# SmoothKen/knn-svc

Measured on AMD Instinct MI355X. Metric: audio-sec converted/sec (xRT) end-to-end, cold target pool, higher is better.
Workload: dtype f32; 1 GPU; north-star point per rank: 30 s source vs 10 min target pool (20 x 30 s), ckpt_type=mix, post_opt_0.2, cold (pool encoded inside the step); seeded random weights of WavLM-Large (6 layers executed) and the 22.9 M-param generator; nq=1500, np_per_rank=30000, wavlm_batch_chunks=32, pipeline_depth=2

## Files before the change

### knn_svc_amd/csrc/attention.hip

```cpp
#include "common.h"
#include "gemm2_core.h"
#include <stdlib.h>

namespace {

constexpr int HD = 64;
constexpr int KT = 64;
constexpr int LDKK = 68;
constexpr int LDV = 64;

__global__ __launch_bounds__(256) void attention_kernel(const float* __restrict__ qkv, const float* __restrict__ gate,
                                                       const float* __restrict__ table, const int* __restrict__ kv_len, int T, int heads,
                                                       float* __restrict__ out) {
    extern __shared__ __attribute__((aligned(16))) float lds[];
    float* Ks = lds;
    float* Vs = Ks + KT * LDKK;
    float* tb = Vs + KT * LDV;

    const int tid = threadIdx.x, lane = tid & 63, wave = tid >> 6;
    const int li = lane & 31, lh = lane >> 5;
    const int head = blockIdx.y, b = blockIdx.z;
    const int E = heads * HD;
    const long ld = 3L * E;
    const float* base = qkv + (long)b * T * ld;
// ... 240 lines not shown
                s = __builtin_amdgcn_mfma_f32_32x32x16_bf16(k0, q2, s, 0, 0, 0);
                s = __builtin_amdgcn_mfma_f32_32x32x16_bf16(k1, q0, s, 0, 0, 0);
                s = __builtin_amdgcn_mfma_f32_32x32x16_bf16(k0, q1, s, 0, 0, 0);
                s = __builtin_amdgcn_mfma_f32_32x32x16_bf16(k0, q0, s, 0, 0, 0);
            }
            const l_f* tp = tbq + kbase;
#pragma unroll
            for (int r = 0; r < 16; ++r) s[r] = fmaf(g_i, tp[(r & 3) + 8 * (r >> 2)], s[r]);
            if (kbase + 32 > Tk) {
#pragma unroll
                for (int r = 0; r < 16; ++r)
                    if (kbase + (r & 3) + 8 * (r >> 2) + 4 * lh >= Tk) s[r] = -__builtin_inff();
            }
            float mx = fmaxf(fmaxf(s[0], s[1]), fmaxf(s[2], s[3]));
#pragma unroll
            for (int r = 4; r < 16; r += 4) mx = fmaxf(mx, fmaxf(fmaxf(s[r], s[r + 1]), fmaxf(s[r + 2], s[r + 3])));
            mx = fmaxf(mx, __shfl_xor(mx, 32, 64));
            const float m_new = fmaxf(m_run, mx);
            const float alpha = __builtin_amdgcn_exp2f(m_run - m_new);
            float ps = 0.f;
#pragma unroll
            for (int r = 0; r < 16; ++r) { s[r] = __builtin_amdgcn_exp2f(s[r] - m_new); ps += s[r]; }
            ps += __shfl_xor(ps, 32, 64);
            l_run = l_run * alpha + ps;
            m_run = m_new;
            if (__builtin_amdgcn_ballot_w64(alpha != 1.f)) {
#pragma unroll
                for (int d = 0; d < 2; ++d)
#pragma unroll
                    for (int r = 0; r < 16; ++r) o[d][r] *= alpha;
            }
#pragma unroll
            for (int st = 0; st < 2; ++st) {
                unsigned h[8], m[8], l[8];
#pragma unroll
                for (int e = 0; e < 8; ++e) split3(s[8 * st + e], h[e], m[e], l[e]);
                au32x4 p0, p1, p2;
#pragma unroll
                for (int w = 0; w < 4; ++w) {
                    p0[w] = pack_hi(h[2 * w + 1], h[2 * w]); p1[w] = pack_hi(m[2 * w + 1], m[2 * w]); p2[w] = pack_hi(l[2 * w + 1], l[2 * w]);
                }
                const bf16x8_t b0 = __builtin_bit_cast(bf16x8_t, p0), b1 = __builtin_bit_cast(bf16x8_t, p1), b2 = __builtin_bit_cast(bf16x8_t, p2);
                const int kcol = (sub * 32 + 16 * st + 4 * lh) * 2;
#pragma unroll
                for (int dt = 0; dt < 2; ++dt) {
                    const lc* vp = Vs + (dt * 32 + li) * VP3 + kcol;
                    au32x4 a0, a1, a2;
                    const au32x2 x0 = *(const l_u2*)(vp), x1 = *(const l_u2*)(vp + 16);
                    const au32x2 y0 = *(const l_u2*)(vp + 128), y1 = *(const l_u2*)(vp + 128 + 16);
                    const au32x2 z0 = *(const l_u2*)(vp + 256), z1 = *(const l_u2*)(vp + 256 + 16);
                    a0 = (au32x4){x0[0], x0[1], x1[0], x1[1]};
                    a1 = (au32x4){y0[0], y0[1], y1[0], y1[1]};
                    a2 = (au32x4){z0[0], z0[1], z1[0], z1[1]};
                    const bf16x8_t v0 = __builtin_bit_cast(bf16x8_t, a0), v1 = __builtin_bit_cast(bf16x8_t, a1), v2 = __builtin_bit_cast(bf16x8_t, a2);
                    f32x16 c = o[dt];
                    c = __builtin_amdgcn_mfma_f32_32x32x16_bf16(v1, b1, c, 0, 0, 0);
                    c = __builtin_amdgcn_mfma_f32_32x32x16_bf16(v2, b0, c, 0, 0, 0);
                    c = __builtin_amdgcn_mfma_f32_32x32x16_bf16(v0, b2, c, 0, 0, 0);
                    c = __builtin_amdgcn_mfma_f32_32x32x16_bf16(v1, b0, c, 0, 0, 0);
                    c = __builtin_amdgcn_mfma_f32_32x32x16_bf16(v0, b1, c, 0, 0, 0);
                    c = __builtin_amdgcn_mfma_f32_32x32x16_bf16(v0, b0, c, 0, 0, 0);
                    o[dt] = c;
                }
            }
        }
    }
    if (qvalid) {
        const float inv = 1.0f / l_run;
        float* op = out + ((long)b * T + qi) * E + head * HD;
#pragma unroll
        for (int d = 0; d < 2; ++d)
#pragma unroll
            for (int r4 = 0; r4 < 4; ++r4) {
                f32x4 v = {o[d][r4 * 4 + 0] * inv, o[d][r4 * 4 + 1] * inv, o[d][r4 * 4 + 2] * inv, o[d][r4 * 4 + 3] * inv};
                *(f32x4*)(op + d * 32 + r4 * 8 + lh * 4) = v;
            }
    }
}

typedef short short4v __attribute__((ext_vector_type(4)));
constexpr int KP2 = 272;
constexpr int VP2 = 320;

__global__ __launch_bounds__(256, 3) void attention2_kernel(const float* __restrict__ qkv, const float* __restrict__ gate,
                                                           const float* __restrict__ table, const int* __restrict__ kv_len, int T, int heads,
                                                           float* __restrict__ out, int out_split, int kv_split) {
    extern __shared__ __attribute__((aligned(16))) float lds[];
    typedef __attribute__((address_space(3))) char lc;
    typedef __attribute__((address_space(3))) au32x4 l_u4;
    typedef __attribute__((address_space(3))) au32x2 l_u2;
    typedef __attribute__((address_space(3))) float l_f;
    lc* Ks = (lc*)lds;
    lc* Vs = Ks + KT * KP2;
    l_f* tb = (l_f*)(Vs + KT * VP2);

    const int tid = threadIdx.x, lane = tid & 63, wave = tid >> 6;
    const int li = lane & 31, lh = lane >> 5;
    const int head = blockIdx.y, b = blockIdx.z;
    const int E = heads * HD;
    const long ld = 3L * E;
    const float* base = qkv + (long)b * T * ld;
    const int qi = blockIdx.x * 128 + wave * 32 + li;
    const bool qvalid = qi < T;
    int Tk = T;
    if (kv_len) { Tk = kv_len[b]; Tk = Tk < 1 ? 1 : (Tk > T ? T : Tk); }

    for (int i = tid; i < 2 * T - 1 + 64; i += 256) tb[i] = i < 2 * T - 1 ? table[(long)head * (2 * T - 1) + i] : 0.f;

    const float L2E = 1.44269504088896341f;
    const float qscale = 0.125f * L2E * 16.0f;
    au32x4 qf[4][2];
#pragma unroll
    for (int s = 0; s < 4; ++s) {
        f32x4 v0 = {0.f, 0.f, 0.f, 0.f}, v1 = v0;
        if (qvalid) {
            const float* p = base + (long)qi * ld + head * HD + s * 16 + lh * 8;
            v0 = *(const f32x4*)p; v1 = *(const f32x4*)(p + 4);
        }
        g2_u32x2 h0, l0, h1, l1;
        f16x2_split4(v0, qscale, h0, l0); f16x2_split4(v1, qscale, h1, l1);
        qf[s][0] = (au32x4){h0[0], h0[1], h1[0], h1[1]};
        qf[s][1] = (au32x4){l0[0], l0[1], l1[0], l1[1]};
    }
    const float g_i = qvalid ? gate[((long)b * T + qi) * heads + head] * (L2E * 256.0f) : 0.f;
    const l_f* tbq = tb + (T - 1 - (qvalid ? qi : T - 1)) + 4 * lh;
    const lc* v_tr = Vs + (4 * (lane >> 5) + ((lane & 15) >> 2)) * VP2 + (16 * ((lane >> 4) & 1) + 4 * (lane & 3)) * 2;


    f32x16 o[2];
#pragma unroll
    for (int d = 0; d < 2; ++d)
#pragma unroll
        for (int r = 0; r < 16; ++r) o[d][r] = 0.f;
    float m_run = -__builtin_inff(), l_run = 0.f;

    const int srow = tid >> 4, scol = (tid & 15) * 4;
    f32x4 rk[4], rv[4];
    auto gload = [&](int k0) {
#pragma unroll
        for (int j = 0; j < 4; ++j) {
            const int key = k0 + srow + 16 * j;
            f32x4 kk = {0.f, 0.f, 0.f, 0.f}, vv = {0.f, 0.f, 0.f, 0.f};
            if (key < T) {
                const float* p = base + (long)key * ld + head * HD + scol;
                kk = *(const f32x4*)(p + E);
                vv = *(const f32x4*)(p + 2 * E);
            }
            rk[j] = kk; rv[j] = vv;
        }
    };
    gload(0);
    const int ntiles = (Tk + KT - 1) / KT;
    for (int t = 0; t < ntiles; ++t) {
#ifdef KN_ATT_NOSTAGE
        if (t == 0) {
#endif
        __syncthreads();
        if (kv_split) {
            const int pc = tid & 15, plane = (pc >> 2) & 1, d0 = (pc >> 3) * 32 + (pc & 3) * 8;
#pragma unroll
            for (int j = 0; j < 4; ++j) {
                const int key = srow + 16 * j;
                *(l_u4*)(Ks + key * KP2 + plane * 128 + d0 * 2) = __builtin_bit_cast(au32x4, rk[j]);
                *(l_u4*)(Vs + key * VP2 + plane * 128 + d0 * 2) = __builtin_bit_cast(au32x4, rv[j]);
            }
        } else {
#pragma unroll
        for (int j = 0; j < 4; ++j) {
            const int key = srow + 16 * j;
            g2_u32x2 hi, lo;
            f16x2_split4(rk[j], 16.0f, hi, lo);
            lc* kd = Ks + key * KP2 + scol * 2;
            *(l_u2*)(kd) = hi;
            *(l_u2*)(kd + 128) = lo;
            f16x2_split4(rv[j], 16.0f, hi, lo);
            lc* vd = Vs + key * VP2 + scol * 2;
            *(l_u2*)(vd) = hi;
            *(l_u2*)(vd + 128) = lo;
        }
        }
        __syncthreads();
#ifdef KN_ATT_NOSTAGE
        }
#else
        if (t + 1 < ntiles) gload((t + 1) * KT);
#endif

#pragma unroll
        for (int sub = 0; sub < 2; ++sub) {
            const int kbase = t * KT + sub * 32;
            if (kbase >= Tk) break;
            f32x16 s;
#pragma unroll
            for (int r = 0; r < 16; ++r) s[r] = 0.f;
            const lc* kp = Ks + (sub * 32 + li) * KP2 + lh * 16;
#pragma unroll
            for (int st = 0; st < 4; ++st) {
                const f16x8 k0 = __builtin_bit_cast(f16x8, *(const l_u4*)(kp + st * 32));
                const f16x8 k1 = __builtin_bit_cast(f16x8, *(const l_u4*)(kp + 128 + st * 32));
                const f16x8 q0 = __builtin_bit_cast(f16x8, qf[st][0]), q1 = __builtin_bit_cast(f16x8, qf[st][1]);
#ifdef KN_ATT_NOS
                if (st == 0) s = __builtin_amdgcn_mfma_f32_32x32x16_f16(k1, q0, s, 0, 0, 0);
                else { s[st] += __builtin_bit_cast(float, __builtin_bit_cast(au32x4, k0)[0] ^ __builtin_bit_cast(au32x4, k1)[1] ^ __builtin_bit_cast(au32x4, q1)[0]); }
#else
                s = __builtin_amdgcn_mfma_f32_32x32x16_f16(k1, q0, s, 0, 0, 0);
                s = __builtin_amdgcn_mfma_f32_32x32x16_f16(k0, q1, s, 0, 0, 0);
                s = __builtin_amdgcn_mfma_f32_32x32x16_f16(k0, q0, s, 0, 0, 0);
#endif
            }
            const l_f* tp = tbq + kbase;
#ifndef KN_ATT_NOBIAS
#pragma unroll
            for (int r = 0; r < 16; ++r) s[r] = fmaf(g_i, tp[(r & 3) + 8 * (r >> 2)], s[r]);
#endif
            if (kbase + 32 > Tk) {
#pragma unroll
                for (int r = 0; r < 16; ++r)
                    if (kbase + (r & 3) + 8 * (r >> 2) + 4 * lh >= Tk) s[r] = -__builtin_inff();
            }
#ifdef KN_ATT_NOEXP
            float mx = s[0];
#else
            float mx = fmaxf(fmaxf(s[0], s[1]), fmaxf(s[2], s[3]));
#pragma unroll
            for (int r = 4; r < 16; r += 4) mx = fmaxf(mx, fmaxf(fmaxf(s[r], s[r + 1]), fmaxf(s[r + 2], s[r + 3])));
#endif
            mx = fmaxf(mx, __shfl_xor(mx, 32, 64));
            const float m_new = fmaxf(m_run, mx);
            const float alpha = __builtin_amdgcn_exp2f((m_run - m_new) * (1.0f / 256.0f));
            const float mneg = fmaf(m_new, -1.0f / 256.0f, 14.0f);
            float ps = 0.f;
#pragma unroll
#ifdef KN_ATT_NOEXP
            for (int r = 0; r < 16; ++r) { s[r] = s[r] * 1e-9f; } ps = s[3] + mneg;
#else
            for (int r = 0; r < 16; ++r) { s[r] = __builtin_amdgcn_exp2f(fmaf(s[r], 1.0f / 256.0f, mneg)); ps += s[r]; }
#endif
            ps += __shfl_xor(ps, 32, 64);
            l_run = l_run * alpha + ps;
            m_run = m_new;
            if (__builtin_amdgcn_ballot_w64(alpha != 1.f)) {
#pragma unroll
                for (int d = 0; d < 2; ++d)
#pragma unroll
                    for (int r = 0; r < 16; ++r) o[d][r] *= alpha;
            }
#pragma unroll
            for (int st = 0; st < 2; ++st) {
                g2_u32x2 h0, l0, h1, l1;
                f16x2_split4((f32x4){s[8 * st + 0], s[8 * st + 1], s[8 * st + 2], s[8 * st + 3]}, 1.0f, h0, l0);
                f16x2_split4((f32x4){s[8 * st + 4], s[8 * st + 5], s[8 * st + 6], s[8 * st + 7]}, 1.0f, h1, l1);
                const f16x8 b0 = __builtin_bit_cast(f16x8, (au32x4){h0[0], h0[1], h1[0], h1[1]});
                const f16x8 b1 = __builtin_bit_cast(f16x8, (au32x4){l0[0], l0[1], l1[0], l1[1]});
                const lc* vrow = v_tr + (sub * 32 + 16 * st) * VP2;
#pragma unroll
                for (int dt = 0; dt < 2; ++dt) {
                    typedef __attribute__((address_space(3))) short4v l_s4;
                    const lc* vp = vrow + dt * 64;
                    const au32x2 x0 = __builtin_bit_cast(au32x2, __builtin_amdgcn_ds_read_tr16_b64_v4i16((l_s4*)(vp)));
                    const au32x2 x1 = __builtin_bit_cast(au32x2, __builtin_amdgcn_ds_read_tr16_b64_v4i16((l_s4*)(vp + 8 * VP2)));
                    const au32x2 y0 = __builtin_bit_cast(au32x2, __builtin_amdgcn_ds_read_tr16_b64_v4i16((l_s4*)(vp + 128)));
                    const au32x2 y1 = __builtin_bit_cast(au32x2, __builtin_amdgcn_ds_read_tr16_b64_v4i16((l_s4*)(vp + 8 * VP2 + 128)));
                    const f16x8 v0 = __builtin_bit_cast(f16x8, (au32x4){x0[0], x0[1], x1[0], x1[1]});
                    const f16x8 v1 = __builtin_bit_cast(f16x8, (au32x4){y0[0], y0[1], y1[0], y1[1]});
                    f32x16 c = o[dt];
#ifdef KN_ATT_NOPV
                    if (dt == 0) c = __builtin_amdgcn_mfma_f32_32x32x16_f16(v1, b0, c, 0, 0, 0);
                    else c[st] += __builtin_bit_cast(float, __builtin_bit_cast(au32x4, v0)[0] ^ __builtin_bit_cast(au32x4, v1)[1] ^ __builtin_bit_cast(au32x4, b1)[0]);
#else
                    c = __builtin_amdgcn_mfma_f32_32x32x16_f16(v1, b0, c, 0, 0, 0);
                    c = __builtin_amdgcn_mfma_f32_32x32x16_f16(v0, b1, c, 0, 0, 0);
                    c = __builtin_amdgcn_mfma_f32_32x32x16_f16(v0, b0, c, 0, 0, 0);
#endif
                    o[dt] = c;
                }
            }
        }
    }
    if (qvalid) {
        const float inv = 0.0625f / l_run;
        float* op = out + ((long)b * T + qi) * E + head * HD;
#pragma unroll
        for (int d = 0; d < 2; ++d)
#pragma unroll
            for (int r4 = 0; r4 < 4; ++r4) {
                f32x4 v = {o[d][r4 * 4 + 0] * inv, o[d][r4 * 4 + 1] * inv, o[d][r4 * 4 + 2] * inv, o[d][r4 * 4 + 3] * inv};
                if (out_split) {
                    g2_u32x2 hi, lo;
                    f16x2_split4(v, KN_F16X2_A_SCALE, hi, lo);
                    const int c = head * HD + d * 32 + r4 * 8 + lh * 4;
                    char* ob = (char*)(out + ((long)b * T + qi) * E) + (c >> 5) * 128 + (c & 31) * 2;
                    *(g2_u32x2*)ob = hi;
                    *(g2_u32x2*)(ob + 64) = lo;
                } else
                    *(f32x4*)(op + d * 32 + r4 * 8 + lh * 4) = v;
            }
    }
}

template <int QB>
__global__ __launch_bounds__(256, 2) void attention2q_kernel(const float* __restrict__ qkv, const float* __restrict__ gate,
                                                            const float* __restrict__ table, const int* __restrict__ kv_len, int T, int heads,
                                                            float* __restrict__ out, int out_split, int kv_split) {
    extern __shared__ __attribute__((aligned(16))) float lds[];
    typedef __attribute__((address_space(3))) char lc;
    typedef __attribute__((address_space(3))) au32x4 l_u4;
    typedef __attribute__((address_space(3))) au32x2 l_u2;
    typedef __attribute__((address_space(3))) float l_f;
    lc* Ks = (lc*)lds;
    lc* Vs = Ks + KT * KP2;
    l_f* tb = (l_f*)(Vs + KT * VP2);

    const int tid = threadIdx.x, lane = tid & 63, wave = tid >> 6;
    const int li = lane & 31, lh = lane >> 5;
    const int head = blockIdx.y, b = blockIdx.z;
    const int E = heads * HD;
    const long ld = 3L * E;
    const float* base = qkv + (long)b * T * ld;
    int Tk = T;
    if (kv_len) { Tk = kv_len[b]; Tk = Tk < 1 ? 1 : (Tk > T ? T : Tk); }

    for (int i = tid; i < 2 * T - 1 + 64; i += 256) tb[i] = i < 2 * T - 1 ? table[(long)head * (2 * T - 1) + i] : 0.f;

    const float L2E = 1.44269504088896341f;
    const float qscale = 0.125f * L2E * 16.0f;
    int qi[QB]; bool qvalid[QB];
    au32x4 qf[QB][4][2];
    float g_i[QB];
    const l_f* tbq[QB];
#pragma unroll
    for (int u = 0; u < QB; ++u) {
        qi[u] = blockIdx.x * (128 * QB) + wave * (32 * QB) + u * 32 + li;
        qvalid[u] = qi[u] < T;
#pragma unroll
        for (int s4 = 0; s4 < 4; ++s4) {
            f32x4 v0 = {0.f, 0.f, 0.f, 0.f}, v1 = v0;
            if (qvalid[u]) {
                const float* p = base + (long)qi[u] * ld + head * HD + s4 * 16 + lh * 8;
                v0 = *(const f32x4*)p; v1 = *(const f32x4*)(p + 4);
            }
            g2_u32x2 h0, l0, h1, l1;
            f16x2_split4(v0, qscale, h0, l0); f16x2_split4(v1, qscale, h1, l1);
            qf[u][s4][0] = (au32x4){h0[0], h0[1], h1[0], h1[1]};
            qf[u][s4][1] = (au32x4){l0[0], l0[1], l1[0], l1[1]};
        }
        g_i[u] = qvalid[u] ? gate[((long)b * T + qi[u]) * heads + head] * (L2E * 256.0f) : 0.f;
        tbq[u] = tb + (T - 1 - (qvalid[u] ? qi[u] : T - 1)) + 4 * lh;
    }
    const lc* v_tr = Vs + (4 * (lane >> 5) + ((lane & 15) >> 2)) * VP2 + (16 * ((lane >> 4) & 1) + 4 * (lane & 3)) * 2;

    f32x16 o[QB][2];
    float m_run[QB], l_run[QB];
#pragma unroll
    for (int u = 0; u < QB; ++u) {
        m_run[u] = -__builtin_inff(); l_run[u] = 0.f;
#pragma unroll
        for (int d = 0; d < 2; ++d)
#pragma unroll
            for (int r = 0; r < 16; ++r) o[u][d][r] = 0.f;
    }

    const int srow = tid >> 4, scol = (tid & 15) * 4;
    f32x4 rk[4], rv[4];
    auto gload = [&](int k0) {
#pragma unroll
        for (int j = 0; j < 4; ++j) {
            const int key = k0 + srow + 16 * j;
            f32x4 kk = {0.f, 0.f, 0.f, 0.f}, vv = {0.f, 0.f, 0.f, 0.f};
            if (key < T) {
                const float* p = base + (long)key * ld + head * HD + scol;
                kk = *(const f32x4*)(p + E);
                vv = *(const f32x4*)(p + 2 * E);
            }
            rk[j] = kk; rv[j] = vv;
        }
    };
    gload(0);
    const int ntiles = (Tk + KT - 1) / KT;
#ifdef KN_ATT_PROF
    unsigned long long pf[4] = {0, 0, 0, 0}, tq = __builtin_readcyclecounter();
    const unsigned long long t_begin = tq;
#define KN_ATICK(K) { const unsigned long long now = __builtin_readcyclecounter(); pf[K] += now - tq; tq = now; }
#else
#define KN_ATICK(K)
#endif
    for (int t = 0; t < ntiles; ++t) {
        __syncthreads();
        if (kv_split) {
            const int pc = tid & 15, plane = (pc >> 2) & 1, d0 = (pc >> 3) * 32 + (pc & 3) * 8;
#pragma unroll
            for (int j = 0; j < 4; ++j) {
                const int key = srow + 16 * j;
                *(l_u4*)(Ks + key * KP2 + plane * 128 + d0 * 2) = __builtin_bit_cast(au32x4, rk[j]);
                *(l_u4*)(Vs + key * VP2 + plane * 128 + d0 * 2) = __builtin_bit_cast(au32x4, rv[j]);
            }
        } else {
#pragma unroll
            for (int j = 0; j < 4; ++j) {
                const int key = srow + 16 * j;
                g2_u32x2 hi, lo;
                f16x2_split4(rk[j], 16.0f, hi, lo);
                lc* kd = Ks + key * KP2 + scol * 2;
                *(l_u2*)(kd) = hi;
                *(l_u2*)(kd + 128) = lo;
                f16x2_split4(rv[j], 16.0f, hi, lo);
                lc* vd = Vs + key * VP2 + scol * 2;
                *(l_u2*)(vd) = hi;
                *(l_u2*)(vd + 128) = lo;
            }
        }
        __syncthreads();
        if (t + 1 < ntiles) gload((t + 1) * KT);
        KN_ATICK(0)

#pragma unroll
        for (int sub = 0; sub < 2; ++sub) {
            const int kbase = t * KT + sub * 32;
            if (kbase >= Tk) break;

            f32x16 s[QB];
#pragma unroll
            for (int u = 0; u < QB; ++u)
#pragma unroll
                for (int r = 0; r < 16; ++r) s[u][r] = 0.f;
            const lc* kp = Ks + (sub * 32 + li) * KP2 + lh * 16;
#pragma unroll
            for (int st = 0; st < 4; ++st) {
                const f16x8 k0 = __builtin_bit_cast(f16x8, *(const l_u4*)(kp + st * 32));
                const f16x8 k1 = __builtin_bit_cast(f16x8, *(const l_u4*)(kp + 128 + st * 32));
#pragma unroll
                for (int u = 0; u < QB; ++u) {
                    const f16x8 q0 = __builtin_bit_cast(f16x8, qf[u][st][0]), q1 = __builtin_bit_cast(f16x8, qf[u][st][1]);
                    s[u] = __builtin_amdgcn_mfma_f32_32x32x16_f16(k1, q0, s[u], 0, 0, 0);
                    s[u] = __builtin_amdgcn_mfma_f32_32x32x16_f16(k0, q1, s[u], 0, 0, 0);
                    s[u] = __builtin_amdgcn_mfma_f32_32x32x16_f16(k0, q0, s[u], 0, 0, 0);
                }
            }
            KN_ATICK(1)
#pragma unroll
            for (int u = 0; u < QB; ++u) {
                const l_f* tp = tbq[u] + kbase;
#pragma unroll
                for (int r = 0; r < 16; ++r) s[u][r] = fmaf(g_i[u], tp[(r & 3) + 8 * (r >> 2)], s[u][r]);
                if (kbase + 32 > Tk) {
#pragma unroll
                    for (int r = 0; r < 16; ++r)
                        if (kbase + (r & 3) + 8 * (r >> 2) + 4 * lh >= Tk) s[u][r] = -__builtin_inff();
                }
                float mx = fmaxf(fmaxf(s[u][0], s[u][1]), fmaxf(s[u][2], s[u][3]));
#pragma unroll
                for (int r = 4; r < 16; r += 4) mx = fmaxf(mx, fmaxf(fmaxf(s[u][r], s[u][r + 1]), fmaxf(s[u][r + 2], s[u][r + 3])));
                mx = fmaxf(mx, __shfl_xor(mx, 32, 64));
                const float m_new = fmaxf(m_run[u], mx);
                const float alpha = __builtin_amdgcn_exp2f((m_run[u] - m_new) * (1.0f / 256.0f));
                const float mneg = fmaf(m_new, -1.0f / 256.0f, 14.0f);
                float ps = 0.f;
#pragma unroll
                for (int r = 0; r < 16; ++r) { s[u][r] = __builtin_amdgcn_exp2f(fmaf(s[u][r], 1.0f / 256.0f, mneg)); ps += s[u][r]; }
                ps += __shfl_xor(ps, 32, 64);
                l_run[u] = l_run[u] * alpha + ps;
                m_run[u] = m_new;
                if (__builtin_amdgcn_ballot_w64(alpha != 1.f)) {
#pragma unroll
                    for (int d = 0; d < 2; ++d)
#pragma unroll
                        for (int r = 0; r < 16; ++r) o[u][d][r] *= alpha;
                }
            }
            KN_ATICK(2)
#pragma unroll
            for (int st = 0; st < 2; ++st) {
                f16x8 b0[QB], b1[QB];
#pragma unroll
                for (int u = 0; u < QB; ++u) {
                    g2_u32x2 h0, l0, h1, l1;
                    f16x2_split4((f32x4){s[u][8 * st + 0], s[u][8 * st + 1], s[u][8 * st + 2], s[u][8 * st + 3]}, 1.0f, h0, l0);
                    f16x2_split4((f32x4){s[u][8 * st + 4], s[u][8 * st + 5], s[u][8 * st + 6], s[u][8 * st + 7]}, 1.0f, h1, l1);
                    b0[u] = __builtin_bit_cast(f16x8, (au32x4){h0[0], h0[1], h1[0], h1[1]});
                    b1[u] = __builtin_bit_cast(f16x8, (au32x4){l0[0], l0[1], l1[0], l1[1]});
                }
                const lc* vrow = v_tr + (sub * 32 + 16 * st) * VP2;
#pragma unroll
                for (int dt = 0; dt < 2; ++dt) {
                    typedef __attribute__((address_space(3))) short4v l_s4;
                    const lc* vp = vrow + dt * 64;
                    const au32x2 x0 = __builtin_bit_cast(au32x2, __builtin_amdgcn_ds_read_tr16_b64_v4i16((l_s4*)(vp)));
                    const au32x2 x1 = __builtin_bit_cast(au32x2, __builtin_amdgcn_ds_read_tr16_b64_v4i16((l_s4*)(vp + 8 * VP2)));
                    const au32x2 y0 = __builtin_bit_cast(au32x2, __builtin_amdgcn_ds_read_tr16_b64_v4i16((l_s4*)(vp + 128)));
                    const au32x2 y1 = __builtin_bit_cast(au32x2, __builtin_amdgcn_ds_read_tr16_b64_v4i16((l_s4*)(vp + 8 * VP2 + 128)));
                    const f16x8 v0 = __builtin_bit_cast(f16x8, (au32x4){x0[0], x0[1], x1[0], x1[1]});
                    const f16x8 v1 = __builtin_bit_cast(f16x8, (au32x4){y0[0], y0[1], y1[0], y1[1]});
#pragma unroll
                    for (int u = 0; u < QB; ++u) {
                        f32x16 c = o[u][dt];
                        c = __builtin_amdgcn_mfma_f32_32x32x16_f16(v1, b0[u], c, 0, 0, 0);
                        c = __builtin_amdgcn_mfma_f32_32x32x16_f16(v0, b1[u], c, 0, 0, 0);
                        c = __builtin_amdgcn_mfma_f32_32x32x16_f16(v0, b0[u], c, 0, 0, 0);
                        o[u][dt] = c;
                    }
                }
            }
            KN_ATICK(3)
        }
    }
#ifdef KN_ATT_PROF
    if (tid == 0 && blockIdx.x == 2 && blockIdx.y == 3 && (blockIdx.z % 5) == 0)
        printf("att prof (cycles per 64-key tile, wave 0 of batch %d): stage+barriers %.0f  S (K reads + issue) %.0f  softmax (incl. wait for S) %.0f  PV (split, V reads, issue) %.0f  | whole block %.0f\n",
               (int)blockIdx.z, (double)pf[0] / ntiles, (double)pf[1] / ntiles, (double)pf[2] / ntiles, (double)pf[3] / ntiles, (double)(__builtin_readcyclecounter() - t_begin));
#endif
#undef KN_ATICK
#pragma unroll
    for (int u = 0; u < QB; ++u) {
        if (!qvalid[u]) continue;
        const float inv = 0.0625f / l_run[u];
        float* op = out + ((long)b * T + qi[u]) * E + head * HD;
#pragma unroll
        for (int d = 0; d < 2; ++d)
#pragma unroll
            for (int r4 = 0; r4 < 4; ++r4) {
                f32x4 v = {o[u][d][r4 * 4 + 0] * inv, o[u][d][r4 * 4 + 1] * inv, o[u][d][r4 * 4 + 2] * inv, o[u][d][r4 * 4 + 3] * inv};
                if (out_split) {
                    g2_u32x2 hi, lo;
                    f16x2_split4(v, KN_F16X2_A_SCALE, hi, lo);
                    const int c = head * HD + d * 32 + r4 * 8 + lh * 4;
                    char* ob = (char*)(out + ((long)b * T + qi[u]) * E) + (c >> 5) * 128 + (c & 31) * 2;
                    *(g2_u32x2*)ob = hi;
                    *(g2_u32x2*)(ob + 64) = lo;
                } else
                    *(f32x4*)(op + d * 32 + r4 * 8 + lh * 4) = v;
            }
    }
}

template <int QB>
__global__ __launch_bounds__(512, 1) void attention2w_kernel(const float* __restrict__ qkv, const float* __restrict__ gate,
                                                            const float* __restrict__ table, const int* __restrict__ kv_len, int T, int heads,
                                                            float* __restrict__ out, int out_split, int kv_split) {
    extern __shared__ __attribute__((aligned(16))) float lds[];
    typedef __attribute__((address_space(3))) char lc;
    typedef __attribute__((address_space(3))) au32x4 l_u4;
    typedef __attribute__((address_space(3))) au32x2 l_u2;
    typedef __attribute__((address_space(3))) float l_f;
    constexpr int NT = 512, NJ = KT * 16 / NT;
    constexpr int KVB = KT * KP2 + KT * VP2;
    lc* Ks = (lc*)lds;
    lc* Vs = Ks + KT * KP2;
    l_f* tb = (l_f*)(Ks + 3 * KVB);

    const int tid = threadIdx.x, lane = tid & 63, wave = __builtin_amdgcn_readfirstlane(tid >> 6);
    const bool late = wave >= 4;
    const int li = lane & 31, lh = lane >> 5;
    const int head = blockIdx.y, b = blockIdx.z;
    const int E = heads * HD;
    const long ld = 3L * E;
    const float* base = qkv + (long)b * T * ld;
    int Tk = T;
    if (kv_len) { Tk = kv_len[b]; Tk = Tk < 1 ? 1 : (Tk > T ? T : Tk); }

    for (int i = tid; i < 2 * T - 1 + 64; i += NT) tb[i] = i < 2 * T - 1 ? table[(long)head * (2 * T - 1) + i] : 0.f;

    const float L2E = 1.44269504088896341f;
    const float qscale = 0.125f * L2E * 16.0f;
    int qi[QB]; bool qvalid[QB];
    au32x4 qf[QB][4][2];
    float g_i[QB];
    const l_f* tbq[QB];
#pragma unroll
    for (int u = 0; u < QB; ++u) {
        qi[u] = blockIdx.x * (8 * 32 * QB) + wave * (32 * QB) + u * 32 + li;
        qvalid[u] = qi[u] < T;
#pragma unroll
        for (int s4 = 0; s4 < 4; ++s4) {
            f32x4 v0 = {0.f, 0.f, 0.f, 0.f}, v1 = v0;
            if (qvalid[u]) {
                const float* p = base + (long)qi[u] * ld + head * HD + s4 * 16 + lh * 8;
                v0 = *(const f32x4*)p; v1 = *(const f32x4*)(p + 4);
            }
            g2_u32x2 h0, l0, h1, l1;
            f16x2_split4(v0, qscale, h0, l0); f16x2_split4(v1, qscale, h1, l1);
            qf[u][s4][0] = (au32x4){h0[0], h0[1], h1[0], h1[1]};
            qf[u][s4][1] = (au32x4){l0[0], l0[1], l1[0], l1[1]};
        }
        g_i[u] = qvalid[u] ? gate[((long)b * T + qi[u]) * heads + head] * (L2E * 256.0f) : 0.f;
        tbq[u] = tb + (T - 1 - (qvalid[u] ? qi[u] : T - 1)) + 4 * lh;
    }
    const lc* v_tr = Vs + (4 * (lane >> 5) + ((lane & 15) >> 2)) * VP2 + (16 * ((lane >> 4) & 1) + 4 * (lane & 3)) * 2;

    f32x16 o[QB][2];
    float m_run[QB], l_run[QB];
#pragma unroll
    for (int u = 0; u < QB; ++u) {
        m_run[u] = -__builtin_inff(); l_run[u] = 0.f;
#pragma unroll
        for (int d = 0; d < 2; ++d)
#pragma unroll
            for (int r = 0; r < 16; ++r) o[u][d][r] = 0.f;
    }

    const int srow = tid >> 4, scol = (tid & 15) * 4;
    f32x4 rk[NJ], rv[NJ];
    auto gload = [&](int k0) {
#pragma unroll
        for (int j = 0; j < NJ; ++j) {
            const int key = k0 + srow + (NT / 16) * j;
            f32x4 kk = {0.f, 0.f, 0.f, 0.f}, vv = {0.f, 0.f, 0.f, 0.f};
            if (key < T) {
                const float* p = base + (long)key * ld + head * HD + scol;
                kk = *(const f32x4*)(p + E);
                vv = *(const f32x4*)(p + 2 * E);
            }
            rk[j] = kk; rv[j] = vv;
        }
    };
    auto stage_tile = [&](int boff) {
        if (kv_split) {
            const int pc = tid & 15, plane = (pc >> 2) & 1, d0 = (pc >> 3) * 32 + (pc & 3) * 8;
#pragma unroll
            for (int j = 0; j < NJ; ++j) {
                const int key = srow + (NT / 16) * j;
                *(l_u4*)(Ks + boff + key * KP2 + plane * 128 + d0 * 2) = __builtin_bit_cast(au32x4, rk[j]);
                *(l_u4*)(Vs + boff + key * VP2 + plane * 128 + d0 * 2) = __builtin_bit_cast(au32x4, rv[j]);
            }
        } else {
#pragma unroll
            for (int j = 0; j < NJ; ++j) {
                const int key = srow + (NT / 16) * j;
                g2_u32x2 hi, lo;
                f16x2_split4(rk[j], 16.0f, hi, lo);
                lc* kd = Ks + boff + key * KP2 + scol * 2;
                *(l_u2*)(kd) = hi;
                *(l_u2*)(kd + 128) = lo;
                f16x2_split4(rv[j], 16.0f, hi, lo);
                lc* vd = Vs + boff + key * VP2 + scol * 2;
                *(l_u2*)(vd) = hi;
                *(l_u2*)(vd + 128) = lo;
            }
        }
    };
    const int ntiles = (Tk + KT - 1) / KT;
    const int nsteps = (Tk + 31) / 32;

    f32x16 s[QB];
    auto do_S = [&](int boff, int sub) {
#pragma unroll
        for (int u = 0; u < QB; ++u)
#pragma unroll
            for (int r = 0; r < 16; ++r) s[u][r] = 0.f;
        const lc* kp = Ks + boff + (sub * 32 + li) * KP2 + lh * 16;
#pragma unroll
        for (int st = 0; st < 4; ++st) {
            const f16x8 k0 = __builtin_bit_cast(f16x8, *(const l_u4*)(kp + st * 32));
            const f16x8 k1 = __builtin_bit_cast(f16x8, *(const l_u4*)(kp + 128 + st * 32));
#pragma unroll
            for (int u = 0; u < QB; ++u) {
                const f16x8 q0 = __builtin_bit_cast(f16x8, qf[u][st][0]), q1 = __builtin_bit_cast(f16x8, qf[u][st][1]);
                s[u] = __builtin_amdgcn_mfma_f32_32x32x16_f16(k1, q0, s[u], 0, 0, 0);
                s[u] = __builtin_amdgcn_mfma_f32_32x32x16_f16(k0, q1, s[u], 0, 0, 0);
                s[u] = __builtin_amdgcn_mfma_f32_32x32x16_f16(k0, q0, s[u], 0, 0, 0);
            }
        }
    };
    auto do_softmax = [&](int g) {
        const int kbase = g * 32;
#pragma unroll
        for (int u = 0; u < QB; ++u) {
            const l_f* tp = tbq[u] + kbase;
#pragma unroll
            for (int r = 0; r < 16; ++r) s[u][r] = fmaf(g_i[u], tp[(r & 3) + 8 * (r >> 2)], s[u][r]);
            if (kbase + 32 > Tk) {
#pragma unroll
                for (int r = 0; r < 16; ++r)
                    if (kbase + (r & 3) + 8 * (r >> 2) + 4 * lh >= Tk) s[u][r] = -__builtin_inff();
            }
            float mx = fmaxf(fmaxf(s[u][0], s[u][1]), fmaxf(s[u][2], s[u][3]));
#pragma unroll
            for (int r = 4; r < 16; r += 4) mx = fmaxf(mx, fmaxf(fmaxf(s[u][r], s[u][r + 1]), fmaxf(s[u][r + 2], s[u][r + 3])));
            mx = fmaxf(mx, __shfl_xor(mx, 32, 64));
            const float m_new = fmaxf(m_run[u], mx);
            const float alpha = __builtin_amdgcn_exp2f((m_run[u] - m_new) * (1.0f / 256.0f));
            const float mneg = fmaf(m_new, -1.0f / 256.0f, 14.0f);
            float ps = 0.f;
#pragma unroll
            for (int r = 0; r < 16; ++r) { s[u][r] = __builtin_amdgcn_exp2f(fmaf(s[u][r], 1.0f / 256.0f, mneg)); ps += s[u][r]; }
            ps += __shfl_xor(ps, 32, 64);
            l_run[u] = l_run[u] * alpha + ps;
            m_run[u] = m_new;
            if (__builtin_amdgcn_ballot_w64(alpha != 1.f)) {
#pragma unroll
                for (int d = 0; d < 2; ++d)
#pragma unroll
                    for (int r = 0; r < 16; ++r) o[u][d][r] *= alpha;
            }
        }
    };
    auto do_PV = [&](int boff, int sub) {
#pragma unroll
        for (int st = 0; st < 2; ++st) {
            f16x8 b0[QB], b1[QB];
#pragma unroll
            for (int u = 0; u < QB; ++u) {
                g2_u32x2 h0, l0, h1, l1;
                f16x2_split4((f32x4){s[u][8 * st + 0], s[u][8 * st + 1], s[u][8 * st + 2], s[u][8 * st + 3]}, 1.0f, h0, l0);
                f16x2_split4((f32x4){s[u][8 * st + 4], s[u][8 * st + 5], s[u][8 * st + 6], s[u][8 * st + 7]}, 1.0f, h1, l1);
                b0[u] = __builtin_bit_cast(f16x8, (au32x4){h0[0], h0[1], h1[0], h1[1]});
                b1[u] = __builtin_bit_cast(f16x8, (au32x4){l0[0], l0[1], l1[0], l1[1]});
            }
            const lc* vrow = v_tr + boff + (sub * 32 + 16 * st) * VP2;
#pragma unroll
            for (int dt = 0; dt < 2; ++dt) {
                typedef __attribute__((address_space(3))) short4v l_s4;
                const lc* vp = vrow + dt * 64;
                const au32x2 x0 = __builtin_bit_cast(au32x2, __builtin_amdgcn_ds_read_tr16_b64_v4i16((l_s4*)(vp)));
                const au32x2 x1 = __builtin_bit_cast(au32x2, __builtin_amdgcn_ds_read_tr16_b64_v4i16((l_s4*)(vp + 8 * VP2)));
                const au32x2 y0 = __builtin_bit_cast(au32x2, __builtin_amdgcn_ds_read_tr16_b64_v4i16((l_s4*)(vp + 128)));
                const au32x2 y1 = __builtin_bit_cast(au32x2, __builtin_amdgcn_ds_read_tr16_b64_v4i16((l_s4*)(vp + 8 * VP2 + 128)));
                const f16x8 v0 = __builtin_bit_cast(f16x8, (au32x4){x0[0], x0[1], x1[0], x1[1]});
                const f16x8 v1 = __builtin_bit_cast(f16x8, (au32x4){y0[0], y0[1], y1[0], y1[1]});
#pragma unroll
                for (int u = 0; u < QB; ++u) {
                    f32x16 c = o[u][dt];
                    c = __builtin_amdgcn_mfma_f32_32x32x16_f16(v1, b0[u], c, 0, 0, 0);
                    c = __builtin_amdgcn_mfma_f32_32x32x16_f16(v0, b1[u], c, 0, 0, 0);
                    c = __builtin_amdgcn_mfma_f32_32x32x16_f16(v0, b0[u], c, 0, 0, 0);
                    o[u][dt] = c;
                }
            }
        }
    };

    gload(0);
    stage_tile(0);
    if (ntiles > 1) { gload(KT); stage_tile(KVB); }
    if (ntiles > 2) gload(2 * KT);
    __syncthreads();
    do_S(0, 0);
    int bc = 0;
    for (int t = 0; t < ntiles; ++t) {
        const int bn = bc == 2 * KVB ? 0 : bc + KVB, bp = bc == 0 ? 2 * KVB : bc - KVB;
        if (t + 2 < ntiles) stage_tile(bp);
        if (t + 3 < ntiles) gload((t + 3) * KT);
        do_softmax(2 * t); do_PV(bc, 0);
        if (2 * t + 1 < nsteps) { do_S(bc, 1); do_softmax(2 * t + 1); do_PV(bc, 1); }
        if (!late) { __builtin_amdgcn_fence(__ATOMIC_RELEASE, "workgroup"); __builtin_amdgcn_s_barrier(); __builtin_amdgcn_fence(__ATOMIC_ACQUIRE, "workgroup"); }
        if (2 * t + 2 < nsteps) do_S(bn, 0);
        if (late) { __builtin_amdgcn_fence(__ATOMIC_RELEASE, "workgroup"); __builtin_amdgcn_s_barrier(); __builtin_amdgcn_fence(__ATOMIC_ACQUIRE, "workgroup"); }
        bc = bn;
    }
#pragma unroll
    for (int u = 0; u < QB; ++u) {
        if (!qvalid[u]) continue;
        const float inv = 0.0625f / l_run[u];
        float* op = out + ((long)b * T + qi[u]) * E + head * HD;
#pragma unroll
        for (int d = 0; d < 2; ++d)
#pragma unroll
            for (int r4 = 0; r4 < 4; ++r4) {
                f32x4 v = {o[u][d][r4 * 4 + 0] * inv, o[u][d][r4 * 4 + 1] * inv, o[u][d][r4 * 4 + 2] * inv, o[u][d][r4 * 4 + 3] * inv};
                if (out_split) {
                    g2_u32x2 hi, lo;
                    f16x2_split4(v, KN_F16X2_A_SCALE, hi, lo);
                    const int c = head * HD + d * 32 + r4 * 8 + lh * 4;
                    char* ob = (char*)(out + ((long)b * T + qi[u]) * E) + (c >> 5) * 128 + (c & 31) * 2;
                    *(g2_u32x2*)ob = hi;
                    *(g2_u32x2*)(ob + 64) = lo;
                } else
                    *(f32x4*)(op + d * 32 + r4 * 8 + lh * 4) = v;
            }
    }
}


}

extern "C" int knnsvc_wavlm_attention(const float* qkv, const float* gate, const float* table, int32_t batches,
                                      int32_t T, int32_t heads, float* out, int32_t out_f16x2, int32_t kv_f16x2, const int32_t* kv_len,
                                      void* stream) {
    KN_REQUIRE(qkv && gate && table && out, "wavlm_attention: null pointer");
    KN_REQUIRE(batches > 0 && T > 0 && heads > 0 && heads <= 65535 && batches <= 65535, "wavlm_attention: bad sizes");
    KN_REQUIRE(((uintptr_t)qkv & 15) == 0 && ((uintptr_t)out & 15) == 0, "wavlm_attention: 16-byte alignment");
    static int env_mode = -1;
    if (env_mode < 0) {
        const char* e = getenv("KNNSVC_ATTENTION");
        env_mode = !e ? 2 : (e[0] == 'b') ? 3 : (e[0] == 'f' && e[1] == 'p') ? 0 : 2;
    }
    const int mode = (out_f16x2 & 4) && env_mode == 2 ? 3 : env_mode;
    out_f16x2 &= 1;
    if (mode == 2) {
        const size_t l2 = (size_t)KT * KP2 + (size_t)KT * VP2 + (size_t)(2 * T - 1 + 64) * 4;
        KN_REQUIRE(l2 <= 160 * 1024, "wavlm_attention: T too long for the LDS bias table (T <= ~16000)");
        static size_t attr2 = 0;
        if (l2 > attr2) {
            if (hipFuncSetAttribute((const void*)attention2_kernel, hipFuncAttributeMaxDynamicSharedMemorySize, (int)l2) != hipSuccess)
                return knnsvc_fail(KNNSVC_EHIP, "wavlm_attention: hipFuncSetAttribute failed");
            attr2 = l2;
        }
        const char* eq = getenv("KNNSVC_ATT_QB");
        const int qb = !eq ? 0 : (eq[0] == '1' ? 1 : 2);
        const long blocks128 = (long)((T + 127) / 128) * heads * batches;
        if ((qb == 2 || (qb == 0 && blocks128 >= 1536)) && T > 128) {
            const char* ew = getenv("KNNSVC_ATT_NW");
            const long blocks512 = (long)((T + 511) / 512) * heads * batches;
            const size_t l2w = (size_t)3 * (KT * KP2 + KT * VP2) + (size_t)(2 * T - 1 + 64) * 4;
            if ((ew ? ew[0] == '8' : blocks512 >= 512) && l2w <= 160 * 1024) {
                static size_t attr2w = 0;
                if (l2w > attr2w) {
                    if (hipFuncSetAttribute((const void*)attention2w_kernel<2>, hipFuncAttributeMaxDynamicSharedMemorySize, (int)l2w) != hipSuccess)
                        return knnsvc_fail(KNNSVC_EHIP, "wavlm_attention: hipFuncSetAttribute failed");
                    attr2w = l2w;
                }
                dim3 gridw((unsigned)((T + 511) / 512), (unsigned)heads, (unsigned)batches);
                hipLaunchKernelGGL(attention2w_kernel<2>, gridw, dim3(512), l2w, (hipStream_t)stream, qkv, gate, table, kv_len, T, heads, out, out_f16x2, kv_f16x2);
                return knnsvc_check_launch("wavlm_attention2w");
            }
            static size_t attr2q = 0;
            if (l2 > attr2q) {
                if (hipFuncSetAttribute((const void*)attention2q_kernel<2>, hipFuncAttributeMaxDynamicSharedMemorySize, (int)l2) != hipSuccess)
                    return knnsvc_fail(KNNSVC_EHIP, "wavlm_attention: hipFuncSetAttribute failed");
                attr2q = l2;
            }
            dim3 gridq((unsigned)((T + 255) / 256), (unsigned)heads, (unsigned)batches);
            hipLaunchKernelGGL(attention2q_kernel<2>, gridq, dim3(256), l2, (hipStream_t)stream, qkv, gate, table, kv_len, T, heads, out, out_f16x2, kv_f16x2);
            return knnsvc_check_launch("wavlm_attention2q");
        }
        dim3 grid2((unsigned)((T + 127) / 128), (unsigned)heads, (unsigned)batches);
        hipLaunchKernelGGL(attention2_kernel, grid2, dim3(256), l2, (hipStream_t)stream, qkv, gate, table, kv_len, T, heads, out, out_f16x2, kv_f16x2);
        return knnsvc_check_launch("wavlm_attention2");
    }
    KN_REQUIRE(!out_f16x2 && !kv_f16x2, "wavlm_attention: split output / pre-split K,V are only implemented by the f16x2 kernel");
    if (mode == 3) {
        const size_t l3 = (size_t)KT * KP3 + (size_t)HD * VP3 + (size_t)(2 * T - 1 + 64) * 4;
        KN_REQUIRE(l3 <= 160 * 1024, "wavlm_attention: T too long for the LDS bias table (T <= ~13000)");
        static size_t attr3 = 0;
        if (l3 > attr3) {
            if (hipFuncSetAttribute((const void*)attention3_kernel, hipFuncAttributeMaxDynamicSharedMemorySize, (int)l3) != hipSuccess)
                return knnsvc_fail(KNNSVC_EHIP, "wavlm_attention: hipFuncSetAttribute failed");
            attr3 = l3;
        }
        dim3 grid3((unsigned)((T + 127) / 128), (unsigned)heads, (unsigned)batches);
        hipLaunchKernelGGL(attention3_kernel, grid3, dim3(256), l3, (hipStream_t)stream, qkv, gate, table, kv_len, T, heads, out);
        return knnsvc_check_launch("wavlm_attention3");
    }
    const size_t lds = (size_t)(KT * LDKK + KT * LDV + 2 * T - 1) * 4;
    KN_REQUIRE(lds <= 160 * 1024, "wavlm_attention: T too long for the LDS bias table (T <= ~16000)");
    static size_t attr = 0;
    if (lds > attr) {
        if (hipFuncSetAttribute((const void*)attention_kernel, hipFuncAttributeMaxDynamicSharedMemorySize, (int)lds) !=
            hipSuccess)
            return knnsvc_fail(KNNSVC_EHIP, "wavlm_attention: hipFuncSetAttribute failed");
        attr = lds;
    }
    dim3 grid((unsigned)((T + 127) / 128), (unsigned)heads, (unsigned)batches);
    hipLaunchKernelGGL(attention_kernel, grid, dim3(256), lds, (hipStream_t)stream, qkv, gate, table, kv_len, T, heads, out);
    return knnsvc_check_launch("wavlm_attention");
}
```

Before: 930.1 x real-time.

## Replicate bias table in shifted copies for vector LDS loads in attention2w

The relative-position bias table in LDS is stored as NC phase-shifted copies, so each lane can read its bias values with aligned vector loads instead of scalar ones. The softmax step and the f16 hi/lo split of P are factored into shared helpers. The split uses an opaque 1.0 and per-element conversion so the compiler emits packed conversions, and late waves get a higher scheduling priority. The cost is more LDS used by the table copies, which lowers the maximum T that takes the wide kernel path. It also adds a second template instantiation.

```diff
diff --git a/knn_svc_amd/csrc/attention.hip b/knn_svc_amd/csrc/attention.hip
--- a/knn_svc_amd/csrc/attention.hip
+++ b/knn_svc_amd/csrc/attention.hip
@@ -346,6 +346,64 @@
 constexpr int KP2 = 272;
 constexpr int VP2 = 320;
 
+__device__ __forceinline__ void att2_softmax_step(f32x16& s, const float (&bias)[16], float g, int kbase, int Tk, int lh,
+                                                  float& m_run, float& l_run, f32x16 (&o)[2]) {
+#ifndef KN_ATT_NOBIAS
+#pragma unroll
+    for (int r = 0; r < 16; ++r) s[r] = fmaf(g, bias[r], s[r]);
+#endif
+    if (kbase + 32 > Tk) {
+#pragma unroll
+        for (int r = 0; r < 16; ++r)
+            if (kbase + (r & 3) + 8 * (r >> 2) + 4 * lh >= Tk) s[r] = -__builtin_inff();
+    }
+#ifdef KN_ATT_NOEXP
+    float mx = s[0];
+#else
+    float mx = fmaxf(s[0], s[1]);
+#pragma unroll
+    for (int r = 2; r < 16; r += 2) mx = fmaxf(fmaxf(mx, s[r]), s[r + 1]);
+#endif
+    const float m_new = fmaxf(fmaxf(m_run, mx), __shfl_xor(mx, 32, 64));
+    const float alpha = __builtin_amdgcn_exp2f((m_run - m_new) * (1.0f / 256.0f));
+    const float mneg = fmaf(m_new, -1.0f / 256.0f, 14.0f);
+    float ps = 0.f;
+#ifdef KN_ATT_NOEXP
+    for (int r = 0; r < 16; ++r) { s[r] = s[r] * 1e-9f; } ps = s[3] + mneg;
+#else
+#pragma unroll
+    for (int r = 0; r < 16; ++r) { s[r] = __builtin_amdgcn_exp2f(fmaf(s[r], 1.0f / 256.0f, mneg)); ps += s[r]; }
+#endif
+    ps += __shfl_xor(ps, 32, 64);
+    l_run = l_run * alpha + ps;
+    m_run = m_new;
+    if (__builtin_amdgcn_ballot_w64(alpha != 1.f)) {
+#pragma unroll
+        for (int d = 0; d < 2; ++d)
+#pragma unroll
+            for (int r = 0; r < 16; ++r) o[d][r] *= alpha;
+    }
+}
+
+__device__ __forceinline__ float att2_opaque_one() {
+    float one = 1.0f;
+    __asm__("" : "+s"(one));
+    return one;
+}
+
+__device__ __forceinline__ void att2_split_p(const f32x16& s, int st, float one, f16x8& b0, f16x8& b1) {
+    f16x8 h, l;
+#pragma unroll
+    for (int e = 0; e < 8; e += 2) {
+        const f32x2_t p = {s[8 * st + e], s[8 * st + e + 1]};
+        const f16x2_t hp = __builtin_convertvector(p, f16x2_t);
+        h[e] = hp[0]; h[e + 1] = hp[1];
+        l[e] = (_Float16)__builtin_fmaf(p[0], one, -(float)hp[0]);
+        l[e + 1] = (_Float16)__builtin_fmaf(p[1], one, -(float)hp[1]);
+    }
+    b0 = h; b1 = l;
+}
+
 __global__ __launch_bounds__(256, 3) void attention2_kernel(const float* __restrict__ qkv, const float* __restrict__ gate,
                                                            const float* __restrict__ table, const int* __restrict__ kv_len, int T, int heads,
                                                            float* __restrict__ out, int out_split, int kv_split) {
@@ -389,7 +447,7 @@
     const float g_i = qvalid ? gate[((long)b * T + qi) * heads + head] * (L2E * 256.0f) : 0.f;
     const l_f* tbq = tb + (T - 1 - (qvalid ? qi : T - 1)) + 4 * lh;
     const lc* v_tr = Vs + (4 * (lane >> 5) + ((lane & 15) >> 2)) * VP2 + (16 * ((lane >> 4) & 1) + 4 * (lane & 3)) * 2;
-
+    const float one = att2_opaque_one();
 
     f32x16 o[2];
 #pragma unroll
@@ -473,49 +531,14 @@
 #endif
             }
             const l_f* tp = tbq + kbase;
-#ifndef KN_ATT_NOBIAS
-#pragma unroll
-            for (int r = 0; r < 16; ++r) s[r] = fmaf(g_i, tp[(r & 3) + 8 * (r >> 2)], s[r]);
-#endif
-            if (kbase + 32 > Tk) {
-#pragma unroll
-                for (int r = 0; r < 16; ++r)
-                    if (kbase + (r & 3) + 8 * (r >> 2) + 4 * lh >= Tk) s[r] = -__builtin_inff();
-            }
-#ifdef KN_ATT_NOEXP
-            float mx = s[0];
-#else
-            float mx = fmaxf(fmaxf(s[0], s[1]), fmaxf(s[2], s[3]));
-#pragma unroll
-            for (int r = 4; r < 16; r += 4) mx = fmaxf(mx, fmaxf(fmaxf(s[r], s[r + 1]), fmaxf(s[r + 2], s[r + 3])));
-#endif
-            mx = fmaxf(mx, __shfl_xor(mx, 32, 64));
-            const float m_new = fmaxf(m_run, mx);
-            const float alpha = __builtin_amdgcn_exp2f((m_run - m_new) * (1.0f / 256.0f));
-            const float mneg = fmaf(m_new, -1.0f / 256.0f, 14.0f);
-            float ps = 0.f;
-#pragma unroll
-#ifdef KN_ATT_NOEXP
-            for (int r = 0; r < 16; ++r) { s[r] = s[r] * 1e-9f; } ps = s[3] + mneg;
-#else
-            for (int r = 0; r < 16; ++r) { s[r] = __builtin_amdgcn_exp2f(fmaf(s[r], 1.0f / 256.0f, mneg)); ps += s[r]; }
-#endif
-            ps += __shfl_xor(ps, 32, 64);
-            l_run = l_run * alpha + ps;
-            m_run = m_new;
-            if (__builtin_amdgcn_ballot_w64(alpha != 1.f)) {
-#pragma unroll
-                for (int d = 0; d < 2; ++d)
-#pragma unroll
-                    for (int r = 0; r < 16; ++r) o[d][r] *= alpha;
-            }
+            float bias[16];
+#pragma unroll
+            for (int r = 0; r < 16; ++r) bias[r] = tp[(r & 3) + 8 * (r >> 2)];
+            att2_softmax_step(s, bias, g_i, kbase, Tk, lh, m_run, l_run, o);
 #pragma unroll
             for (int st = 0; st < 2; ++st) {
-                g2_u32x2 h0, l0, h1, l1;
-                f16x2_split4((f32x4){s[8 * st + 0], s[8 * st + 1], s[8 * st + 2], s[8 * st + 3]}, 1.0f, h0, l0);
-                f16x2_split4((f32x4){s[8 * st + 4], s[8 * st + 5], s[8 * st + 6], s[8 * st + 7]}, 1.0f, h1, l1);
-                const f16x8 b0 = __builtin_bit_cast(f16x8, (au32x4){h0[0], h0[1], h1[0], h1[1]});
-                const f16x8 b1 = __builtin_bit_cast(f16x8, (au32x4){l0[0], l0[1], l1[0], l1[1]});
+                f16x8 b0, b1;
+                att2_split_p(s, st, one, b0, b1);
                 const lc* vrow = v_tr + (sub * 32 + 16 * st) * VP2;
 #pragma unroll
                 for (int dt = 0; dt < 2; ++dt) {
@@ -612,6 +635,7 @@
         tbq[u] = tb + (T - 1 - (qvalid[u] ? qi[u] : T - 1)) + 4 * lh;
     }
     const lc* v_tr = Vs + (4 * (lane >> 5) + ((lane & 15) >> 2)) * VP2 + (16 * ((lane >> 4) & 1) + 4 * (lane & 3)) * 2;
+    const float one = att2_opaque_one();
 
     f32x16 o[QB][2];
     float m_run[QB], l_run[QB];
@@ -704,45 +728,17 @@
 #pragma unroll
             for (int u = 0; u < QB; ++u) {
                 const l_f* tp = tbq[u] + kbase;
-#pragma unroll
-                for (int r = 0; r < 16; ++r) s[u][r] = fmaf(g_i[u], tp[(r & 3) + 8 * (r >> 2)], s[u][r]);
-                if (kbase + 32 > Tk) {
-#pragma unroll
-                    for (int r = 0; r < 16; ++r)
-                        if (kbase + (r & 3) + 8 * (r >> 2) + 4 * lh >= Tk) s[u][r] = -__builtin_inff();
-                }
-                float mx = fmaxf(fmaxf(s[u][0], s[u][1]), fmaxf(s[u][2], s[u][3]));
-#pragma unroll
-                for (int r = 4; r < 16; r += 4) mx = fmaxf(mx, fmaxf(fmaxf(s[u][r], s[u][r + 1]), fmaxf(s[u][r + 2], s[u][r + 3])));
-                mx = fmaxf(mx, __shfl_xor(mx, 32, 64));
-                const float m_new = fmaxf(m_run[u], mx);
-                const float alpha = __builtin_amdgcn_exp2f((m_run[u] - m_new) * (1.0f / 256.0f));
-                const float mneg = fmaf(m_new, -1.0f / 256.0f, 14.0f);
-                float ps = 0.f;
-#pragma unroll
-                for (int r = 0; r < 16; ++r) { s[u][r] = __builtin_amdgcn_exp2f(fmaf(s[u][r], 1.0f / 256.0f, mneg)); ps += s[u][r]; }
-                ps += __shfl_xor(ps, 32, 64);
-                l_run[u] = l_run[u] * alpha + ps;
-                m_run[u] = m_new;
-                if (__builtin_amdgcn_ballot_w64(alpha != 1.f)) {
-#pragma unroll
-                    for (int d = 0; d < 2; ++d)
-#pragma unroll
-                        for (int r = 0; r < 16; ++r) o[u][d][r] *= alpha;
-                }
+                float bias[16];
+#pragma unroll
+                for (int r = 0; r < 16; ++r) bias[r] = tp[(r & 3) + 8 * (r >> 2)];
+                att2_softmax_step(s[u], bias, g_i[u], kbase, Tk, lh, m_run[u], l_run[u], o[u]);
             }
             KN_ATICK(2)
 #pragma unroll
             for (int st = 0; st < 2; ++st) {
                 f16x8 b0[QB], b1[QB];
 #pragma unroll
-                for (int u = 0; u < QB; ++u) {
-                    g2_u32x2 h0, l0, h1, l1;
-                    f16x2_split4((f32x4){s[u][8 * st + 0], s[u][8 * st + 1], s[u][8 * st + 2], s[u][8 * st + 3]}, 1.0f, h0, l0);
-                    f16x2_split4((f32x4){s[u][8 * st + 4], s[u][8 * st + 5], s[u][8 * st + 6], s[u][8 * st + 7]}, 1.0f, h1, l1);
-                    b0[u] = __builtin_bit_cast(f16x8, (au32x4){h0[0], h0[1], h1[0], h1[1]});
-                    b1[u] = __builtin_bit_cast(f16x8, (au32x4){l0[0], l0[1], l1[0], l1[1]});
-                }
+                for (int u = 0; u < QB; ++u) att2_split_p(s[u], st, one, b0[u], b1[u]);
                 const lc* vrow = v_tr + (sub * 32 + 16 * st) * VP2;
 #pragma unroll
                 for (int dt = 0; dt < 2; ++dt) {
@@ -796,7 +792,9 @@
     }
 }
 
-template <int QB>
+__host__ __device__ __forceinline__ int att2w_tb_pitch(int T, int NC) { return (2 * T - 1 + 64 - 64 / NC + 63) / 64 * 64 + 64 / NC; }
+
+template <int QB, int NC>
 __global__ __launch_bounds__(512, 1) void attention2w_kernel(const float* __restrict__ qkv, const float* __restrict__ gate,
                                                             const float* __restrict__ table, const int* __restrict__ kv_len, int T, int heads,
                                                             float* __restrict__ out, int out_split, int kv_split) {
@@ -807,9 +805,10 @@
     typedef __attribute__((address_space(3))) float l_f;
     constexpr int NT = 512, NJ = KT * 16 / NT;
     constexpr int KVB = KT * KP2 + KT * VP2;
-    lc* Ks = (lc*)lds;
+    const int tbp = att2w_tb_pitch(T, NC);
+    l_f* tb = (l_f*)lds;
+    lc* Ks = (lc*)(tb + NC * tbp);
     lc* Vs = Ks + KT * KP2;
-    l_f* tb = (l_f*)(Ks + 3 * KVB);
 
     const int tid = threadIdx.x, lane = tid & 63, wave = __builtin_amdgcn_readfirstlane(tid >> 6);
     const bool late = wave >= 4;
@@ -821,7 +820,8 @@
     int Tk = T;
     if (kv_len) { Tk = kv_len[b]; Tk = Tk < 1 ? 1 : (Tk > T ? T : Tk); }
 
-    for (int i = tid; i < 2 * T - 1 + 64; i += NT) tb[i] = i < 2 * T - 1 ? table[(long)head * (2 * T - 1) + i] : 0.f;
+    for (int c = 0; c < NC; ++c)
+        for (int i = tid; i < tbp; i += NT) tb[c * tbp + i] = i + c < 2 * T - 1 ? table[(long)head * (2 * T - 1) + i + c] : 0.f;
 
     const float L2E = 1.44269504088896341f;
     const float qscale = 0.125f * L2E * 16.0f;
@@ -846,9 +846,11 @@
             qf[u][s4][1] = (au32x4){l0[0], l0[1], l1[0], l1[1]};
         }
         g_i[u] = qvalid[u] ? gate[((long)b * T + qi[u]) * heads + head] * (L2E * 256.0f) : 0.f;
-        tbq[u] = tb + (T - 1 - (qvalid[u] ? qi[u] : T - 1)) + 4 * lh;
+        const int toff = (T - 1 - (qvalid[u] ? qi[u] : T - 1)) + 4 * lh, ph = toff & (NC - 1);
+        tbq[u] = tb + ph * tbp + (toff - ph);
     }
     const lc* v_tr = Vs + (4 * (lane >> 5) + ((lane & 15) >> 2)) * VP2 + (16 * ((lane >> 4) & 1) + 4 * (lane & 3)) * 2;
+    const float one = att2_opaque_one();
 
     f32x16 o[QB][2];
     float m_run[QB], l_run[QB];
@@ -928,33 +930,19 @@
         const int kbase = g * 32;
 #pragma unroll
         for (int u = 0; u < QB; ++u) {
+            typedef float fnc __attribute__((ext_vector_type(NC)));
+            typedef __attribute__((address_space(3))) fnc l_fnc;
             const l_f* tp = tbq[u] + kbase;
-#pragma unroll
-            for (int r = 0; r < 16; ++r) s[u][r] = fmaf(g_i[u], tp[(r & 3) + 8 * (r >> 2)], s[u][r]);
-            if (kbase + 32 > Tk) {
-#pragma unroll
-                for (int r = 0; r < 16; ++r)
-                    if (kbase + (r & 3) + 8 * (r >> 2) + 4 * lh >= Tk) s[u][r] = -__builtin_inff();
-            }
-            float mx = fmaxf(fmaxf(s[u][0], s[u][1]), fmaxf(s[u][2], s[u][3]));
-#pragma unroll
-            for (int r = 4; r < 16; r += 4) mx = fmaxf(mx, fmaxf(fmaxf(s[u][r], s[u][r + 1]), fmaxf(s[u][r + 2], s[u][r + 3])));
-            mx = fmaxf(mx, __shfl_xor(mx, 32, 64));
-            const float m_new = fmaxf(m_run[u], mx);
-            const float alpha = __builtin_amdgcn_exp2f((m_run[u] - m_new) * (1.0f / 256.0f));
-            const float mneg = fmaf(m_new, -1.0f / 256.0f, 14.0f);
-            float ps = 0.f;
-#pragma unroll
-            for (int r = 0; r < 16; ++r) { s[u][r] = __builtin_amdgcn_exp2f(fmaf(s[u][r], 1.0f / 256.0f, mneg)); ps += s[u][r]; }
-            ps += __shfl_xor(ps, 32, 64);
-            l_run[u] = l_run[u] * alpha + ps;
-            m_run[u] = m_new;
-            if (__builtin_amdgcn_ballot_w64(alpha != 1.f)) {
-#pragma unroll
-                for (int d = 0; d < 2; ++d)
-#pragma unroll
-                    for (int r = 0; r < 16; ++r) o[u][d][r] *= alpha;
-            }
+            float bias[16];
+#pragma unroll
+            for (int j = 0; j < 4; ++j)
+#pragma unroll
+                for (int h = 0; h < 4; h += NC) {
+                    const fnc v = *(const l_fnc*)(tp + 8 * j + h);
+#pragma unroll
+                    for (int e = 0; e < NC; ++e) bias[4 * j + h + e] = v[e];
+                }
+            att2_softmax_step(s[u], bias, g_i[u], kbase, Tk, lh, m_run[u], l_run[u], o[u]);
         }
     };
     auto do_PV = [&](int boff, int sub) {
@@ -962,13 +950,7 @@
         for (int st = 0; st < 2; ++st) {
             f16x8 b0[QB], b1[QB];
 #pragma unroll
-            for (int u = 0; u < QB; ++u) {
-                g2_u32x2 h0, l0, h1, l1;
-                f16x2_split4((f32x4){s[u][8 * st + 0], s[u][8 * st + 1], s[u][8 * st + 2], s[u][8 * st + 3]}, 1.0f, h0, l0);
-                f16x2_split4((f32x4){s[u][8 * st + 4], s[u][8 * st + 5], s[u][8 * st + 6], s[u][8 * st + 7]}, 1.0f, h1, l1);
-                b0[u] = __builtin_bit_cast(f16x8, (au32x4){h0[0], h0[1], h1[0], h1[1]});
-                b1[u] = __builtin_bit_cast(f16x8, (au32x4){l0[0], l0[1], l1[0], l1[1]});
-            }
+            for (int u = 0; u < QB; ++u) att2_split_p(s[u], st, one, b0[u], b1[u]);
             const lc* vrow = v_tr + boff + (sub * 32 + 16 * st) * VP2;
 #pragma unroll
             for (int dt = 0; dt < 2; ++dt) {
@@ -997,6 +979,7 @@
     if (ntiles > 1) { gload(KT); stage_tile(KVB); }
     if (ntiles > 2) gload(2 * KT);
     __syncthreads();
+    if (late) __builtin_amdgcn_s_setprio(1);
     do_S(0, 0);
     int bc = 0;
     for (int t = 0; t < ntiles; ++t) {
@@ -1064,16 +1047,23 @@
         if ((qb == 2 || (qb == 0 && blocks128 >= 1536)) && T > 128) {
             const char* ew = getenv("KNNSVC_ATT_NW");
             const long blocks512 = (long)((T + 511) / 512) * heads * batches;
-            const size_t l2w = (size_t)3 * (KT * KP2 + KT * VP2) + (size_t)(2 * T - 1 + 64) * 4;
-            if ((ew ? ew[0] == '8' : blocks512 >= 512) && l2w <= 160 * 1024) {
-                static size_t attr2w = 0;
-                if (l2w > attr2w) {
-                    if (hipFuncSetAttribute((const void*)attention2w_kernel<2>, hipFuncAttributeMaxDynamicSharedMemorySize, (int)l2w) != hipSuccess)
+            const size_t kv3 = (size_t)3 * (KT * KP2 + KT * VP2);
+            const size_t l2w4 = kv3 + (size_t)4 * att2w_tb_pitch(T, 4) * 4, l2w2 = kv3 + (size_t)2 * att2w_tb_pitch(T, 2) * 4;
+            if ((ew ? ew[0] == '8' : blocks512 >= 512) && l2w2 <= 160 * 1024) {
+                const bool nc4 = l2w4 <= 160 * 1024;
+                const size_t l2w = nc4 ? l2w4 : l2w2;
+                const void* kw = nc4 ? (const void*)attention2w_kernel<2, 4> : (const void*)attention2w_kernel<2, 2>;
+                static size_t attr2w[2] = {0, 0};
+                if (l2w > attr2w[nc4]) {
+                    if (hipFuncSetAttribute(kw, hipFuncAttributeMaxDynamicSharedMemorySize, (int)l2w) != hipSuccess)
                         return knnsvc_fail(KNNSVC_EHIP, "wavlm_attention: hipFuncSetAttribute failed");
-                    attr2w = l2w;
+                    attr2w[nc4] = l2w;
                 }
                 dim3 gridw((unsigned)((T + 511) / 512), (unsigned)heads, (unsigned)batches);
-                hipLaunchKernelGGL(attention2w_kernel<2>, gridw, dim3(512), l2w, (hipStream_t)stream, qkv, gate, table, kv_len, T, heads, out, out_f16x2, kv_f16x2);
+                if (nc4)
+                    hipLaunchKernelGGL((attention2w_kernel<2, 4>), gridw, dim3(512), l2w, (hipStream_t)stream, qkv, gate, table, kv_len, T, heads, out, out_f16x2, kv_f16x2);
+                else
+                    hipLaunchKernelGGL((attention2w_kernel<2, 2>), gridw, dim3(512), l2w, (hipStream_t)stream, qkv, gate, table, kv_len, T, heads, out, out_f16x2, kv_f16x2);
                 return knnsvc_check_launch("wavlm_attention2w");
             }
             static size_t attr2q = 0;
```

After: 931.9 x real-time, median of 6. No clear change (+0.2%).
